# bootphon/abnet3

Hardware: AMD Instinct MI355X
Metric: frame-pairs/sec (Siamese train step: fwd both towers + coscos2 + bwd + Adadelta) (higher is better)
Workload: dtype f16x2; 1 GPU; C2: SiameseNetwork 40->500x2->100 sigmoid, coscos2(avg=False), Adadelta(0.1), 4096 frame pairs per GPU per step, 40-d N(0,1) frames; pairs_per_gpu=4096, global_pairs=4096, parallelism=dp1, graph_replay=False, dp_gradient_buckets=1

## Files before the change

### abnet3_amd/csrc/common.h

```cpp
#pragma once
#include <hip/hip_runtime.h>
#include <stdint.h>
#include <stdio.h>

#include "../../include/abnet3_hip.h"

namespace abn {

void set_error(const char* fmt, ...);

#define ABN_REQUIRE(cond, ...)                      \
    do {                                            \
        if (!(cond)) {                              \
            ::abn::set_error(__VA_ARGS__);          \
            return ABN_E_ARG;                       \
        }                                           \
    } while (0)

#define ABN_CHECK_LAUNCH(what)                                               \
    do {                                                                     \
        hipError_t e_ = hipGetLastError();                                   \
        if (e_ != hipSuccess) {                                              \
            ::abn::set_error("%s: %s", what, hipGetErrorString(e_));         \
            return ABN_E_LAUNCH;                                             \
// ... 3 lines not shown
struct Switches {
    bool planes;
    bool fused;
    int64_t fused_min_rows;
    bool bn_planes;
    bool bn_persist;
    bool wgrad_xcd;
    bool bf16x3_planes;
    bool bwd_pair;
    int gemm_tile;
    bool dtw_f40, dtw_pc;
    int wgrad_tile128;
    int dtw_wgs_per_cu;
    int wgrad_wgs_heavy, wgrad_wgs_light;
    int64_t wgrad_rows_per_slab;
    bool wide;
    int64_t wide_max_rows;
    int wide_max_groups;
    bool wgrad_step;
    bool dtw_dealt;
    int oneshot_wgs;
    int knn_split;
    int sd_tiles;
};
const Switches& switches();
void reload_switches();

__device__ __forceinline__ bool abn_ticket_publish(double* slot, double value, unsigned* counter, unsigned n_tickets)
{
    __hip_atomic_store(slot, value, __ATOMIC_RELAXED, __HIP_MEMORY_SCOPE_AGENT);
#ifdef ABN_STRICT_FENCES
    const unsigned ticket = __hip_atomic_fetch_add(counter, 1u, __ATOMIC_ACQ_REL, __HIP_MEMORY_SCOPE_AGENT);
#else
    __atomic_signal_fence(__ATOMIC_SEQ_CST);
    __builtin_amdgcn_s_waitcnt(0);
    __atomic_signal_fence(__ATOMIC_SEQ_CST);
    const unsigned ticket = __hip_atomic_fetch_add(counter, 1u, __ATOMIC_RELAXED, __HIP_MEMORY_SCOPE_AGENT);
#endif
    return ticket == n_tickets - 1;
}
__device__ __forceinline__ double abn_ticket_partial(const double* slot)
{
    return __hip_atomic_load(slot, __ATOMIC_RELAXED, __HIP_MEMORY_SCOPE_AGENT);
}

static inline int64_t align_up(int64_t v, int64_t a) { return (v + a - 1) / a * a; }
// ... 18 lines not shown
```

### abnet3_amd/csrc/tower.hip

```cpp
#include <stdarg.h>
#include <stdlib.h>
#include <string.h>

#include <math.h>
#include <atomic>

#include "common.h"
#include "gemm_f32.h"
#include "opt_rule.h"
#include "tower_fused.h"
#include "tower_planes.h"
#include "tower_bn_persist.h"
#include "tower_wide.h"
#include "tower_wgrad_step.h"

namespace abn {

static thread_local char g_err[512] = "";
void set_error(const char* fmt, ...)
{
    va_list ap;
    va_start(ap, fmt);
    vsnprintf(g_err, sizeof(g_err), fmt, ap);
    va_end(ap);
}

static Switches read_switches()
{
    auto off = [](const char* name) { const char* v = getenv(name); return v && atoi(v) == 0; };
    Switches s;
    s.planes = !off("ABN_PLANES");
    s.fused = !off("ABN_FUSED");
    s.fused_min_rows = getenv("ABN_FUSED_MIN_ROWS") ? atoll(getenv("ABN_FUSED_MIN_ROWS")) : -1;
// ... 3 lines not shown
    s.bf16x3_planes = !off("ABN_BF16X3_PLANES");
    s.bwd_pair = !off("ABN_BWD_PAIR");
    s.gemm_tile = getenv("ABN_GEMM_TILE") ? atoi(getenv("ABN_GEMM_TILE")) : -1;
    s.wgrad_rows_per_slab = getenv("ABN_WGRAD_ROWS_PER_SLAB") ? atoll(getenv("ABN_WGRAD_ROWS_PER_SLAB")) : -1;
    s.wide = !off("ABN_WIDE");
    s.wide_max_rows = getenv("ABN_WIDE_MAX_ROWS") ? atoll(getenv("ABN_WIDE_MAX_ROWS")) : -1;
    s.wide_max_groups = getenv("ABN_WIDE_MAXG") ? atoi(getenv("ABN_WIDE_MAXG")) : WD_MAXG;
    if (s.wide_max_groups < 1 || s.wide_max_groups > WD_MAXG) s.wide_max_groups = WD_MAXG;
    s.dtw_f40 = !off("ABN_DTW_F40");
    s.dtw_pc = !off("ABN_DTW_PC");
    s.wgrad_wgs_heavy = getenv("ABN_WGRAD_WGS_HEAVY") ? atoi(getenv("ABN_WGRAD_WGS_HEAVY")) : 128;
    s.wgrad_wgs_light = getenv("ABN_WGRAD_WGS_LIGHT") ? atoi(getenv("ABN_WGRAD_WGS_LIGHT")) : 128;
    s.wgrad_tile128 = getenv("ABN_WGRAD_TILE128") ? atoi(getenv("ABN_WGRAD_TILE128")) : -1;
    s.dtw_wgs_per_cu = getenv("ABN_DTW_WGS") ? atoi(getenv("ABN_DTW_WGS")) : 6;
    if (s.dtw_wgs_per_cu < 1 || s.dtw_wgs_per_cu > 9) s.dtw_wgs_per_cu = 6;
    s.wgrad_step = !off("ABN_WGRAD_STEP");
    s.dtw_dealt = !off("ABN_DTW_SCHED");
    s.oneshot_wgs = getenv("ABN_ONESHOT_WGS") ? atoi(getenv("ABN_ONESHOT_WGS")) : 32;
    if (s.oneshot_wgs < 1 || s.oneshot_wgs > 256) s.oneshot_wgs = 32;
    s.knn_split = getenv("ABN_KNN_SPLIT") ? atoi(getenv("ABN_KNN_SPLIT")) : 0;
    if (s.knn_split < 0) s.knn_split = 0;
    s.sd_tiles = getenv("ABN_SD_TILES") ? atoi(getenv("ABN_SD_TILES")) : 0;
    if (s.sd_tiles < 0 || s.sd_tiles > 4096) s.sd_tiles = 0;
    return s;
}
static Switches g_switches = read_switches();
const Switches& switches() { return g_switches; }
void reload_switches() { g_switches = read_switches(); }

#ifdef ABN_STAMPS
static unsigned long long* stamp_buffer(const char* name)
{
    const char* v = getenv(name);
    return v ? (unsigned long long*)strtoull(v, nullptr, 0) : nullptr;
}
#endif

template <int BM, int BN, bool A_KC, bool B_KC, int EPI, bool VEC, int BF16>
static void launch_one(const GemmP& p, int splits, hipStream_t st)
{
    const int tiles = ((p.M + BM - 1) / BM) * ((p.N + BN - 1) / BN);
    constexpr size_t lds = BF16 == 3 ? gemm_lds_bytes3<BM, BN>() : gemm_lds_bytes<BM, BN, A_KC, B_KC>();
    auto k = gemm_f32_kernel<BM, BN, A_KC, B_KC, EPI, VEC, BF16>;
    static bool attr_set[16] = {};
    if (first_use_on_device(attr_set))
        (void)hipFuncSetAttribute(reinterpret_cast<const void*>(k), hipFuncAttributeMaxDynamicSharedMemorySize, (int)lds);
// ... 154 lines not shown
    GemmP p = {};
    p.A = dz; p.lda = N;
    p.B = a_in; p.ldb = K;
    p.C = slabs; p.ldc = K;
    p.C2 = slabs + N * K;
    p.slab_stride = slab_stride;
    p.M = (int)N; p.N = (int)K + 1; p.K = (int)rows;
    p.k_chunk = (int)align_up((rows + splits - 1) / splits, BK);
    p.ones_col = (int)K;
    p.a_vec = vec_ok(dz, N);
    p.b_vec = vec_ok(a_in, K);
    p.bf16 = prec;
    return p;
}

__global__ void act_bwd_kernel(const float* __restrict__ a, const float* __restrict__ da,
                               const float* __restrict__ mask, float* __restrict__ dz, int64_t n, int act)
{
    for (int64_t i = blockIdx.x * (int64_t)blockDim.x + threadIdx.x; i < n;
         i += (int64_t)gridDim.x * blockDim.x)
        dz[i] = da[i] * act_grad(a[i], act) * (mask ? mask[i] : 1.0f);
}

struct ReduceTable {
    int n_layers;
    int splits[ABN_MAX_LAYERS];
    int64_t slab_stride;
    int64_t off[ABN_MAX_LAYERS];
    int64_t nW[ABN_MAX_LAYERS];
    int64_t nb[ABN_MAX_LAYERS];
    float* dW[ABN_MAX_LAYERS];
    float* db[ABN_MAX_LAYERS];
    int64_t total;
    int64_t begin;
    int n_extra;
    int64_t extra_off[2 * ABN_MAX_LAYERS];
    int32_t extra_n[2 * ABN_MAX_LAYERS];
    const unsigned* fail_word;
    int n_own;
    float* own[2 * ABN_MAX_LAYERS];
    int32_t own_n[2 * ABN_MAX_LAYERS];
};

__device__ __forceinline__ f32x4 sum_slabs(const float* __restrict__ src, int S, int64_t stride)
{
    f32x4 p[4] = {{0.f, 0.f, 0.f, 0.f}, {0.f, 0.f, 0.f, 0.f}, {0.f, 0.f, 0.f, 0.f}, {0.f, 0.f, 0.f, 0.f}};
    int k = 0;
    for (; k + 15 < S; k += 16) {
        f32x4 v[16];
#pragma unroll
        for (int u = 0; u < 16; ++u) v[u] = *reinterpret_cast<const f32x4*>(src + (int64_t)(k + u) * stride);
#pragma unroll
        for (int u = 0; u < 16; ++u) p[u & 3] += v[u];
    }
    for (; k + 3 < S; k += 4) {
        f32x4 v[4];
#pragma unroll
        for (int u = 0; u < 4; ++u) v[u] = *reinterpret_cast<const f32x4*>(src + (int64_t)(k + u) * stride);
#pragma unroll
        for (int u = 0; u < 4; ++u) p[u] += v[u];
    }
    for (; k < S; ++k) p[0] += *reinterpret_cast<const f32x4*>(src + (int64_t)k * stride);
    return (p[0] + p[1]) + (p[2] + p[3]);
}

__global__ void slab_reduce_kernel(const float* __restrict__ slabs, ReduceTable t)
{
    const bool dropped = t.fail_word && *t.fail_word != 0u;
    if (dropped && blockIdx.x == 0)
        for (int k = 0; k < t.n_own; ++k)
            for (int i = threadIdx.x; i < t.own_n[k]; i += blockDim.x) t.own[k][i] = 0.0f;
    const int64_t n4 = (t.total + 3) / 4;
    for (int64_t q = t.begin / 4 + blockIdx.x * (int64_t)blockDim.x + threadIdx.x; q < n4;
         q += (int64_t)gridDim.x * blockDim.x) {
        const int64_t i = 4 * q;
        int l = 0;
        while (l + 1 < t.n_layers && i >= t.off[l + 1]) ++l;
        const int S = t.splits[l];
        const f32x4 s = dropped ? f32x4{0.0f, 0.0f, 0.0f, 0.0f} : sum_slabs(slabs + i, S, t.slab_stride);
#pragma unroll
        for (int e = 0; e < 4; ++e) {
            const int64_t j = i + e - t.off[l];
            if (j < t.nW[l]) t.dW[l][j] = s[e];
            else if (j - t.nW[l] < t.nb[l]) t.db[l][j - t.nW[l]] = s[e];
        }
    }
}

__global__ void slab_reduce_step_kernel(const float* __restrict__ slabs, ReduceTable t, OptP o, float* __restrict__ params,
                                        float* __restrict__ grads, float* __restrict__ s1, float* __restrict__ s2,
                                        const unsigned* __restrict__ fail_word, int32_t* __restrict__ step_ctr)
{
    if (step_ctr && blockIdx.x == 0 && threadIdx.x == 0) *step_ctr += 1;
    if (fail_word && *fail_word != 0u) return;
    const int64_t n4 = (t.total + 3) / 4;
    for (int64_t q = blockIdx.x * (int64_t)blockDim.x + threadIdx.x; q < n4;
         q += (int64_t)gridDim.x * blockDim.x) {
        const int64_t i = 4 * q;
        int l = 0;
        while (l + 1 < t.n_layers && i >= t.off[l + 1]) ++l;
        const int S = t.splits[l];
        const int64_t baseW = t.dW[l] - grads, baseb = t.db[l] - grads;
        const int64_t j0 = i - t.off[l];
        const bool inW = j0 + 3 < t.nW[l], inb = j0 >= t.nW[l] && (j0 - t.nW[l]) + 3 < t.nb[l];
        const int64_t idx0 = inW ? baseW + j0 : baseb + (j0 - t.nW[l]);
        if ((inW || inb) && (idx0 & 3) == 0) {
            f32x4 pv = *reinterpret_cast<const f32x4*>(params + idx0);
            f32x4 av = *reinterpret_cast<const f32x4*>(s1 + idx0);
            f32x4 bv = {0.f, 0.f, 0.f, 0.f};
            if (opt_uses_s2(o)) bv = *reinterpret_cast<const f32x4*>(s2 + idx0);
            const f32x4 s = sum_slabs(slabs + i, S, t.slab_stride);
#pragma unroll
            for (int e = 0; e < 4; ++e) {
                float a1 = av[e], a2 = bv[e];
                pv[e] = opt_update_reg(o, pv[e], s[e], a1, a2);
                av[e] = a1; bv[e] = a2;
            }
            *reinterpret_cast<f32x4*>(grads + idx0) = s;
            *reinterpret_cast<f32x4*>(params + idx0) = pv;
            *reinterpret_cast<f32x4*>(s1 + idx0) = av;
            if (opt_uses_s2(o)) *reinterpret_cast<f32x4*>(s2 + idx0) = bv;
            continue;
        }
        const f32x4 s = sum_slabs(slabs + i, S, t.slab_stride);
#pragma unroll
        for (int e = 0; e < 4; ++e) {
            const int64_t j = j0 + e;
            int64_t idx;
            if (j < t.nW[l]) idx = baseW + j;
            else if (j - t.nW[l] < t.nb[l]) idx = baseb + (j - t.nW[l]);
            else continue;
            grads[idx] = s[e];
            params[idx] = opt_update(o, params[idx], s[e], s1, s2, idx);
        }
    }
    for (int x = 0; x < t.n_extra; ++x)
        for (int64_t j = blockIdx.x * (int64_t)blockDim.x + threadIdx.x; j < t.extra_n[x]; j += (int64_t)gridDim.x * blockDim.x) {
            const int64_t idx = t.extra_off[x] + j;
            params[idx] = opt_update(o, params[idx], grads[idx], s1, s2, idx);
        }
}


constexpr int BN_MAX_CHUNKS = 128;
static inline int bn_chunks(int64_t rows_per_call)
{
    const int64_t c = (rows_per_call + 63) / 64;
    return (int)(c < 1 ? 1 : (c > BN_MAX_CHUNKS ? BN_MAX_CHUNKS : c));
}
static inline int64_t bn_chunk_rows(int64_t rows_per_call) { return (rows_per_call + bn_chunks(rows_per_call) - 1) / bn_chunks(rows_per_call); }

template <bool BWD>
__global__ __launch_bounds__(256) void bn_partial_kernel(const float* __restrict__ z ,
                                                         const float* __restrict__ a, const float* __restrict__ xhat,
                                                         int64_t rows_per_call, int C, int64_t chunk_rows, int act,
                                                         double* __restrict__ part)
{
// ... 755 lines not shown
    ReduceTable rt = {};
    const int nl = t->n_layers;
    rt.n_layers = nl;
    rt.slab_stride = B.slab_stride;
    for (int l = 0; l < nl; ++l) {
        rt.splits[l] = B.splits[l];
        rt.off[l] = B.off[l];
        rt.nW[l] = t->dims[l + 1] * t->dims[l];
        rt.nb[l] = t->dims[l + 1];
        rt.dW[l] = t->dW[l];
        rt.db[l] = t->db[l];
    }
    rt.total = B.off[nl - 1] + rt.nW[nl - 1] + rt.nb[nl - 1];
    if (t->batch_norm && t->sync_ws) {
        rt.fail_word = reinterpret_cast<const unsigned*>(t->sync_ws) + 16;
        for (int l = 0; l < nl; ++l) {
            if (t->dbn_w[l]) { rt.own[rt.n_own] = t->dbn_w[l]; rt.own_n[rt.n_own++] = (int32_t)rt.nb[l]; }
            if (t->dbn_b[l]) { rt.own[rt.n_own] = t->dbn_b[l]; rt.own_n[rt.n_own++] = (int32_t)rt.nb[l]; }
        }
    }
    return rt;
}

static void reduce_one_layer(const float* slabs, int64_t slab_stride, int splits, int64_t in_dim, int64_t out_dim, float* dW, float* db,
                             hipStream_t st)
{
    ReduceTable rt = {};
    rt.n_layers = 1; rt.splits[0] = splits; rt.slab_stride = slab_stride;
    rt.off[0] = 0; rt.nW[0] = out_dim * in_dim; rt.nb[0] = out_dim; rt.dW[0] = dW; rt.db[0] = db;
    rt.total = out_dim * in_dim + out_dim;
    hipLaunchKernelGGL(slab_reduce_kernel, dim3(grid_for((rt.total + 3) / 4)), dim3(256), 0, st, slabs, rt);
}

static void bn_layer_backward(const abn_tower_desc* t, int l, int act, const float* da, float* dz, int64_t rows, int64_t n_calls,
                              const Layout& L, const BwdLayout& B, const float* ws, float* scratch, hipStream_t st)
{
    const int C = (int)t->dims[l + 1];
    const int64_t rpc = rows / n_calls;
    const float* a = ws + L.a[l];
    const int nch = bn_chunks(rpc);
    double* part = reinterpret_cast<double*>(scratch + B.bn_part);
    hipLaunchKernelGGL(bn_partial_kernel<true>, dim3((C + 63) / 64, nch, (int)n_calls), dim3(256), 0, st, da, a,
                       ws + L.xhat[l], rpc, C, bn_chunk_rows(rpc), act, part);
    hipLaunchKernelGGL(bn_bwd_finish_kernel, dim3((unsigned)((n_calls * C + 63) / 64)), dim3(64), 0, st, part,
                       nch, C, (int)n_calls, scratch + B.bn_s1, scratch + B.bn_s2);
    hipLaunchKernelGGL(bn_bwd_apply_kernel, dim3(grid_for(rows * C)), dim3(256), 0, st, a, da,
                       ws + L.xhat[l], rows, rpc, C, act, t->bn_w[l], ws + L.invstd[l], scratch + B.bn_s1, scratch + B.bn_s2,
                       (int)n_calls, t->drop_mask[l], dz, t->dbn_w[l], t->dbn_b[l]);
}

struct LossArgs {
    const void* y;
    int y_dtype, kind, avg;
    float margin;
// ... 45 lines not shown
    }
    *n_wg_out = n_wg;
    return w;
}

static int wgrad_range(const abn_tower_desc* t, int* l_first, int* l_end)
{
    *l_first = 0; *l_end = t->n_layers;
    if (t->wgrad_part == 0) return ABN_OK;
    ABN_REQUIRE(t->wgrad_part == 1 || t->wgrad_part == 2, "tower_backward: wgrad_part=%d", t->wgrad_part);
    ABN_REQUIRE(t->wgrad_split >= 0 && t->wgrad_split <= t->n_layers, "tower_backward: wgrad_split=%d", t->wgrad_split);
    ABN_REQUIRE(!t->defer_reduce, "tower_backward: wgrad_part cannot be combined with defer_reduce");
    if (t->wgrad_part == 1) *l_first = t->wgrad_split;
    else *l_end = t->wgrad_split;
    return ABN_OK;
}
static int reduce_slabs(const abn_tower_desc* t, const BwdLayout& B, const float* scratch, int l_first, int l_end, hipStream_t st)
{
    if (t->defer_reduce) return ABN_OK;
    ReduceTable rt = make_reduce_table(t, B);
    rt.begin = B.off[l_first < t->n_layers ? l_first : t->n_layers - 1];
    if (l_first >= t->n_layers) rt.begin = rt.total;
    if (l_end < t->n_layers) rt.total = B.off[l_end];
    if (rt.total > rt.begin)
        hipLaunchKernelGGL(slab_reduce_kernel, dim3(grid_for((rt.total - rt.begin + 3) / 4)), dim3(256), 0, st, scratch + B.slabs, rt);
    ABN_CHECK_LAUNCH("slab_reduce");
    return ABN_OK;
}

static int bn_planes_backward(const abn_tower_desc* t, const float* d_out, const LossArgs* loss, int64_t rows, int64_t n_calls, const Layout& L,
                              const BwdLayout& B0, const float* ws, float* scratch, float* dx, hipStream_t st)
{
    const int nl = t->n_layers;
    const int np = planes_of(t);
    const int64_t rpc = rows / n_calls;
    ABN_REQUIRE(aligned16(d_out) && aligned16(scratch) && (!dx || aligned16(dx)), "tower_backward: d_out / scratch / dx must be 16-byte aligned");
    ABN_REQUIRE(!t->d_out_is_dz || loss, "tower_backward: d_out_is_dz cannot be combined with batch_norm");
    ABN_REQUIRE(!loss || n_calls == 2, "tower_backward_loss: two forward_once calls");
    BwdLayout B = B0;
    for (int l = 0; l < nl; ++l) B.splits[l] = B0.psplits[l];
    const PackLayout PL = make_pack_layout(t);
    const char* const image = t->wpack ? reinterpret_cast<const char*>(t->wpack) : reinterpret_cast<const char*>(ws + L.wpack);
    static bool attr_set[16] = {};
    if (first_use_on_device(attr_set)) {
        PL_LDS_ATTR(bn_bwd_layer_kernel, pl_lds_bytes);
        PL_LDS_ATTR(wgrad_planes_kernel, wgrad_lds_of);
    }
    const int wgs_per_call = (int)bn_wgs_per_call(rows, n_calls);
// ... 256 lines not shown
                    q.y = t->source->labels;
                    q.g_steps = t->source->steps; q.g_ctr = t->source->step_ctr;
                }
            }
        }
        const dim3 grid((unsigned)(nrb * q.G));
        PL_LAUNCH(np, wide_dgrad_layer_kernel, grid, dim3(PL_NT), wd_lds_bytes(np), st, q);
        if (l < top || q.dz_out) cur ^= (q.dz_out ? 1 : 0);
        if (l == 0) break;
    }
    if (wgrad_step_small_ok(t, rows, n_calls)) {
        ABN_REQUIRE(t->fwd_ws == ws && t->fwd_calls == n_calls, "tower_backward: abn_tower_desc.fwd_ws / fwd_calls are not this call's");
        ABN_CHECK_LAUNCH("tower_backward (layer per launch)");
        return ABN_OK;
    }
    int n_wg = 0;
    WgradP w = make_wgrad(t, rows, L, B, ws, scratch, &n_wg, l_first, l_end);
    w.tp_steps = 2 * nrb;
    if (n_wg > 0) launch_wgrad(np, w, n_wg, st);
    ABN_CHECK_LAUNCH("tower_backward (layer per launch)");
    return reduce_slabs(t, B, scratch, l_first, l_end, st);
}

static int make_planes_fwd(const abn_tower_desc* t, const float* x1, const float* x2, int64_t rows, int64_t n_calls, int train,
                           const Layout& L, float* ws, hipStream_t st, PlanesFwdP* out)
{
    const int np = planes_of(t);
    PackTable pk = {};
    PlanesFwdP f = {};
    f.n_layers = t->n_layers;
    f.rows = (int)rows;
    f.rows_call = (int)(rows / n_calls);
    f.x1 = x1; f.x2 = x2;
    f.x_copy = nullptr;
    const PackLayout PL = make_pack_layout(t);
    char* const image = t->wpack ? reinterpret_cast<char*>(t->wpack) : reinterpret_cast<char*>(ws + L.wpack);
    const bool repack = !(t->wpack && t->wpack_valid);
    ABN_REQUIRE(aligned16(image), "tower_forward: wpack must be 16-byte aligned");
    pk.base = image;
    f.wbase = image; f.wbytes = PL.bytes;
    for (int l = 0; l <= t->n_layers; ++l) f.dims[l] = (int)t->dims[l];
    for (int l = 0; l < t->n_layers; ++l) {
        f.act[l] = (l == t->n_layers - 1) ? t->last_act : t->act;
        f.b[l] = t->b[l];
        f.mask[l] = train ? t->drop_mask[l] : nullptr;
        f.out[l] = l == t->n_layers - 1 ? ws + L.a[l] : nullptr;
        f.wp[l] = image + PL.wp[l];
        PackJob& J = pk.job[pk.n_jobs++];
        J.W = t->W[l]; J.N = (int)t->dims[l + 1]; J.K = (int)t->dims[l]; J.transposed = 0;
        J.nblk = pl_blocks(J.N); J.nsteps = pl_steps(J.K);
        J.tile0 = pk.n_tiles; J.dst = PL.wp[l];
        J.blk0 = pk.n_blocks;
        pk.n_tiles += J.nblk * J.nsteps;
        pk.n_blocks += J.nblk;
        {
            PackJob& T = pk.job[pk.n_jobs++];
            T.W = t->W[l]; T.N = J.N; T.K = J.K; T.transposed = 1;
            T.nblk = pl_blocks(T.K); T.nsteps = pl_steps(T.N);
            T.tile0 = pk.n_tiles; T.dst = PL.wpt[l];
            T.blk0 = pk.n_blocks;
            pk.n_tiles += T.nblk * T.nsteps;
            pk.n_blocks += T.nblk;
        }
        f.tp[l] = (t->forward_only || t->batch_norm) ? nullptr : reinterpret_cast<char*>(ws + L.tp[l]);
        f.amax[l] = f.tp[l] && L.amax[l] >= 0 ? ws + L.amax[l] : nullptr;
        if (t->batch_norm) { f.bn_rm[l] = t->bn_rm[l]; f.bn_rv[l] = t->bn_rv[l]; f.bn_w[l] = t->bn_w[l]; f.bn_b[l] = t->bn_b[l]; }
    }
    f.tp_steps = pl_row_steps(rows);
    f.drop_seed = train ? reinterpret_cast<const unsigned long long*>(t->drop_seed) : nullptr;
    f.drop_p = t->drop_p;
    f.bn_eps = BN_EPS;
#ifdef ABN_STAMPS
    f.stamps = stamp_buffer("ABN_STAMP_BUF");
#endif
    if (repack) {
        const dim3 pgrid((unsigned)((pk.n_tiles + 3) / 4));
        if (np == 3) hipLaunchKernelGGL(pack_planes_kernel<3>, pgrid, dim3(256), 0, st, pk);
        else if (np == 2) hipLaunchKernelGGL(pack_planes_scaled_kernel, dim3((unsigned)pk.n_blocks), dim3(PL_NT), 0, st, pk);
        else hipLaunchKernelGGL(pack_planes_kernel<1>, pgrid, dim3(256), 0, st, pk);
    }
    *out = f;
    return ABN_OK;
}

static int wide_forward(const abn_tower_desc* t, const float* x1, const float* x2, int64_t rows, int64_t n_calls, int train,
                        const Layout& L, float* ws, hipStream_t st)
{
    PlanesFwdP f;
    { const int rc = make_planes_fwd(t, x1, x2, rows, n_calls, train, L, ws, st, &f); if (rc != ABN_OK) return rc; }
    const int np = planes_of(t);
    static bool wd_attr_set[16] = {};
    if (first_use_on_device(wd_attr_set)) PL_LDS_ATTR(wide_fwd_layer_kernel, wd_lds_bytes);
    const int nl = t->n_layers;
    const int64_t wpc = bn_wgs_per_call(rows, n_calls), nrb = n_calls * wpc;
    const int G = wide_groups_for(t, nrb * PL_ROWS);
    const bool keep = !t->forward_only;
    for (int l = 0; l < nl; ++l) {
        WideFwdP q = {};
        q.l = l; q.last = l == nl - 1;
        q.K = (int)t->dims[l]; q.N = (int)t->dims[l + 1];
        q.act = f.act[l];
// ... 567 lines not shown
            if (hipFuncSetAttribute(reinterpret_cast<const void*>(wgrad_step_small_kernel), hipFuncAttributeMaxDynamicSharedMemorySize, (int)WGS_LDS_BYTES) != hipSuccess) {
                set_error("tower_reduce_step: cannot reserve %zu bytes of LDS", WGS_LDS_BYTES);
                return ABN_E_LAUNCH;
            }
            wgs_attr[dev] = true;
        }
        hipLaunchKernelGGL(wgrad_step_small_kernel, dim3((unsigned)n_wg), dim3(WGS_NT), WGS_LDS_BYTES, (hipStream_t)stream, w);
        ABN_CHECK_LAUNCH("tower_reduce_step (weight gradients + step)");
        return ABN_OK;
    }
    ReduceTable rt = make_reduce_table(t, B);
    for (int l = 0; l < t->n_layers; ++l) {
        ABN_REQUIRE(t->dW[l] && t->db[l] && t->dW[l] >= grads && t->dW[l] + rt.nW[l] <= grads + n && t->db[l] >= grads &&
                        t->db[l] + rt.nb[l] <= grads + n,
                    "tower_reduce_step: layer %d's gradients are not inside the flat buffer", l);
        if (t->batch_norm) {
            ABN_REQUIRE(t->dbn_w[l] && t->dbn_b[l] && t->dbn_w[l] >= grads && t->dbn_w[l] + rt.nb[l] <= grads + n &&
                            t->dbn_b[l] >= grads && t->dbn_b[l] + rt.nb[l] <= grads + n,
                        "tower_reduce_step: layer %d's BatchNorm gradients are not inside the flat buffer", l);
            rt.extra_off[rt.n_extra] = t->dbn_w[l] - grads; rt.extra_n[rt.n_extra++] = (int32_t)rt.nb[l];
            rt.extra_off[rt.n_extra] = t->dbn_b[l] - grads; rt.extra_n[rt.n_extra++] = (int32_t)rt.nb[l];
        }
    }
    hipLaunchKernelGGL(slab_reduce_step_kernel, dim3(grid_for((rt.total + 3) / 4)), dim3(256), 0, (hipStream_t)stream,
                       scratch + B.slabs, rt, make_optp(kind, lr, hp0, hp1, eps, step, grad_scale), params, grads, state1,
                       state2, t->batch_norm && t->sync_ws ? reinterpret_cast<const unsigned*>(t->sync_ws) + 16 : nullptr,
                       t->source ? t->source->step_ctr : nullptr);
    ABN_CHECK_LAUNCH("tower_reduce_step");
    return ABN_OK;
}


int abn_linear_forward(const float* x, const float* W, const float* b, int64_t rows, int64_t in_dim,
                       int64_t out_dim, int act, float* y, void* stream)
{
    ABN_REQUIRE(x && W && y, "linear_forward: null pointer");
    ABN_REQUIRE(rows >= 0 && rows < (1LL << 30) && in_dim >= 1 && out_dim >= 1 && in_dim < (1 << 24) && out_dim < (1 << 24),
                "linear_forward: bad shape");
    ABN_REQUIRE(act >= ABN_ACT_NONE && act <= ABN_ACT_TANH, "linear_forward: unsupported activation %d", act);
    const GemmP p = fwd_gemm(x, W, b, y, rows, in_dim, out_dim, act, nullptr, 0);
    return launch_gemm<true, true, EPI_FWD>(p, 1, (hipStream_t)stream);
}

int abn_linear_dgrad(const float* dz, const float* W, int64_t rows, int64_t in_dim, int64_t out_dim,
                     const float* a_prev, int act_prev, float* dx, void* stream)
{
    ABN_REQUIRE(dz && W && dx, "linear_dgrad: null pointer");
    ABN_REQUIRE(rows >= 0 && rows < (1LL << 30) && in_dim >= 1 && out_dim >= 1 && in_dim < (1 << 24) && out_dim < (1 << 24),
                "linear_dgrad: bad shape");
    ABN_REQUIRE(act_prev >= ABN_ACT_NONE && act_prev <= ABN_ACT_TANH, "linear_dgrad: unsupported activation %d", act_prev);
// ... 67 lines not shown
```

### abnet3_amd/csrc/tower_planes.h

```cpp
#pragma once
#include <type_traits>

#include "gemm_f32.h"

namespace abn {

typedef int v4i __attribute__((ext_vector_type(4)));

constexpr int PL_ROWS = 32;
constexpr int PL_WAVES = 8;
constexpr int PL_NT = 64 * PL_WAVES;
constexpr int PL_MAXW = 512;
constexpr int PL_MAXSTEPS = PL_MAXW / 16;
#ifdef PL_DEPTH_OVERRIDE
constexpr int PL_DEPTH = PL_DEPTH_OVERRIDE;
#else
constexpr int PL_DEPTH = 4;
#endif
constexpr int PL_PART_BYTES = 4 * 16 * 64 * 4;
constexpr int PL_SC_BYTES = PL_WAVES * 64 * 4 + PL_WAVES * 32 * 4;
constexpr int PL_AMAX = 32;

__host__ __device__ inline int pl_steps(int64_t contraction) { return ((int)((contraction + 15) / 16) + PL_DEPTH - 1) / PL_DEPTH * PL_DEPTH; }
__host__ __device__ inline int pl_blocks(int64_t features) { return (int)((features + 31) / 32); }
// ... 184 lines not shown
template <int NP>
__device__ __forceinline__ int tgather_row_offset(int r)
{
    const int sp = r >> 4, jh = (r >> 3) & 1, jl = r & 3, hp = (r >> 2) & 1;
    if constexpr (NP >= 2) return sp * 2048 + jh * 1024 + hp * 32 * 16 + jl * 4;
    else return sp * 1024 + hp * 32 * 16 + (4 * jh + jl) * 2;
}
template <int NP>
__device__ __forceinline__ float tgather(const char* tile_pair, int row_off, int c)
{
    if constexpr (NP >= 2) return *reinterpret_cast<const float*>(tile_pair + row_off + c * 16);
    else return (float)*reinterpret_cast<const __bf16*>(tile_pair + row_off + c * 16);
}

template <int N> __device__ __forceinline__ void wait_vmcnt() { asm volatile("s_waitcnt vmcnt(%0)" :: "n"(N) : "memory"); }

struct PackJob {
    const float* W;
    int N, K;
    int transposed;
    int nblk, nsteps;
    int tile0;
    int blk0;
    int64_t dst;
};
struct PackTable {
    int n_jobs, n_tiles, n_blocks;
    char* base;
    PackJob job[2 * ABN_MAX_LAYERS];
};

template <int NP>
__global__ __launch_bounds__(256) void pack_planes_kernel(PackTable t)
{
    const int tile = __builtin_amdgcn_readfirstlane(blockIdx.x * 4 + (threadIdx.x >> 6));
    if (tile >= t.n_tiles) return;
    const int lane = threadIdx.x & 63, r = lane & 31, h = lane >> 5;
    int jn = 0;
    while (jn + 1 < t.n_jobs && tile >= t.job[jn + 1].tile0) ++jn;
    const PackJob& J = t.job[jn];
    const int local = tile - J.tile0;
    const int nb = local / J.nsteps, s = local % J.nsteps;
    const int a = 32 * nb + r;
    const int rows_a = J.transposed ? J.K : J.N;
    const int len_c = J.transposed ? J.N : J.K;
    f32x4 v0 = {0.f, 0.f, 0.f, 0.f}, v1 = v0;
    if (a < rows_a) {
        const int c0 = 16 * s + 4 * h, c1 = c0 + 8;
        if (!J.transposed) {
            if (c0 < len_c) v0 = *reinterpret_cast<const f32x4*>(J.W + (int64_t)a * J.K + c0);
            if (c1 < len_c) v1 = *reinterpret_cast<const f32x4*>(J.W + (int64_t)a * J.K + c1);
        } else {
#pragma unroll
            for (int e = 0; e < 4; ++e) {
                if (c0 + e < len_c) v0[e] = J.W[(int64_t)(c0 + e) * J.K + a];
                if (c1 + e < len_c) v1[e] = J.W[(int64_t)(c1 + e) * J.K + a];
            }
        }
    }
    write_frag<NP>(t.base + J.dst + ((int64_t)local * NP) * 1024 + lane * 16, v0, v1);
}

__global__ __launch_bounds__(PL_NT) void pack_planes_scaled_kernel(PackTable t)
{
    __shared__ float wmax[PL_WAVES];
    const int lane = threadIdx.x & 63, r = lane & 31, h = lane >> 5;
    const int wave = __builtin_amdgcn_readfirstlane(threadIdx.x >> 6);
    const int b = blockIdx.x;
    int jn = 0;
    while (jn + 1 < t.n_jobs && b >= t.job[jn + 1].blk0) ++jn;
    const PackJob& J = t.job[jn];
    const int nb = b - J.blk0;
    const int rows_a = J.transposed ? J.K : J.N;
    const int len_c = J.transposed ? J.N : J.K;
    const int a = 32 * nb + r;
    const int ac = a < rows_a ? a : rows_a - 1;
    constexpr int SPW = PL_MAXSTEPS / PL_WAVES;
    f32x4 v[SPW][2];
    float m = 0.0f;
#pragma unroll
    for (int i = 0; i < SPW; ++i) {
        const int s = wave + PL_WAVES * i;
        const bool live = s < J.nsteps && a < rows_a;
#pragma unroll
        for (int u = 0; u < 2; ++u) {
            const int c = 16 * s + 4 * h + 8 * u;
            const int cc = c < len_c ? c : len_c - 4;
            f32x4 x;
            if (!J.transposed) {
                x = *reinterpret_cast<const f32x4*>(J.W + (int64_t)ac * J.K + cc);
            } else {
#pragma unroll
                for (int e = 0; e < 4; ++e) x[e] = J.W[(int64_t)(cc + e) * J.K + ac];
            }
            const bool ok = live && c < len_c;
#pragma unroll
            for (int e = 0; e < 4; ++e) v[i][u][e] = ok ? x[e] : 0.0f;
        }
        m = fmaxf(m, absmax8(v[i][0], v[i][1]));
    }
    m = wave_max(m);
    if (lane == 0) wmax[wave] = m;
    __syncthreads();
#pragma unroll
    for (int w = 0; w < PL_WAVES; ++w) m = fmaxf(m, wmax[w]);
    float sc, inv;
    scale_of(m, sc, inv);
    char* const image = t.base + J.dst;
#pragma unroll
    for (int i = 0; i < SPW; ++i) {
        const int s = wave + PL_WAVES * i;
        if (s < J.nsteps) write_frag<2>(image + ((int64_t)(nb * J.nsteps + s) * 2) * 1024 + lane * 16, v[i][0], v[i][1], sc);
    }
    if (threadIdx.x == 0) reinterpret_cast<float*>(image + (int64_t)J.nblk * J.nsteps * 2048)[nb] = inv;
}
__device__ __forceinline__ float packed_inv(const char* __restrict__ image, int nblk, int nsteps, int blk)
{
    return reinterpret_cast<const float*>(image + (int64_t)nblk * nsteps * 2048)[blk < nblk ? blk : nblk - 1];
}

#ifdef PL_HANDOVER_ON
constexpr bool PL_HANDOVER = true;
#else
constexpr bool PL_HANDOVER = false;
#endif
#ifndef PL_THROTTLE_LAG
#define PL_THROTTLE_LAG 0
#endif
#ifndef PL_THROTTLE_NAP
#define PL_THROTTLE_NAP 2
#endif
template <int NP>
struct WeightRing {
    __amdgpu_buffer_rsrc_t rs;
    v4i wq[PL_DEPTH][2][NP];
    bool filled;
};
// ... 1910 lines not shown
```

Measured before the change: 26.03 million frame-pairs/s.

## Rework slab reduction into per-wave chunks and split scaled weight packing across workgroups

The slab reduce and reduce+optimizer-step kernels now assign fixed 256-float chunks to waves. Segments are sorted by split count, and templated batch loads are specialized by slab count, so the per-element layer search goes away and loads can be issued together. The scaled weight-pack kernel is split into multiple workgroups per block. Its transposed path now reads coalesced rows and transposes through LDS, where it previously used strided scalar loads. Each part recomputes the full block absmax, which duplicates read work. Legacy paths and timing stamps remain available behind env switches.

```diff
diff --git a/abnet3_amd/csrc/common.h b/abnet3_amd/csrc/common.h
--- a/abnet3_amd/csrc/common.h
+++ b/abnet3_amd/csrc/common.h
@@ -49,6 +49,10 @@
     int oneshot_wgs;
     int knn_split;
     int sd_tiles;
+    bool pack_legacy;
+    int pack_split;
+    bool reduce_legacy;
+    int reduce_wgs;
 };
 const Switches& switches();
 void reload_switches();
diff --git a/abnet3_amd/csrc/tower.hip b/abnet3_amd/csrc/tower.hip
--- a/abnet3_amd/csrc/tower.hip
+++ b/abnet3_amd/csrc/tower.hip
@@ -9,6 +9,7 @@
 #include "gemm_f32.h"
 #include "opt_rule.h"
 #include "tower_fused.h"
+#include <climits>
 #include "tower_planes.h"
 #include "tower_bn_persist.h"
 #include "tower_wide.h"
@@ -58,6 +59,12 @@
     if (s.knn_split < 0) s.knn_split = 0;
     s.sd_tiles = getenv("ABN_SD_TILES") ? atoi(getenv("ABN_SD_TILES")) : 0;
     if (s.sd_tiles < 0 || s.sd_tiles > 4096) s.sd_tiles = 0;
+    s.pack_legacy = getenv("ABN_PACK_LEGACY") && atoi(getenv("ABN_PACK_LEGACY")) == 1;
+    s.pack_split = getenv("ABN_PACK_SPLIT") ? atoi(getenv("ABN_PACK_SPLIT")) : 4;
+    if (s.pack_split != 1 && s.pack_split != 2 && s.pack_split != 4) s.pack_split = 4;
+    s.reduce_legacy = getenv("ABN_REDUCE_LEGACY") && atoi(getenv("ABN_REDUCE_LEGACY")) == 1;
+    s.reduce_wgs = getenv("ABN_REDUCE_WGS") ? atoi(getenv("ABN_REDUCE_WGS")) : 4;
+    if (s.reduce_wgs < 1 || s.reduce_wgs > 16) s.reduce_wgs = 4;
     return s;
 }
 static Switches g_switches = read_switches();
@@ -258,6 +265,15 @@
         dz[i] = da[i] * act_grad(a[i], act) * (mask ? mask[i] : 1.0f);
 }
 
+struct ReduceSeg {
+    int64_t off;
+    int64_t nW, nb;
+    float* dW;
+    float* db;
+    int S;
+    int chunk0;
+    int64_t pad[2];
+};
 struct ReduceTable {
     int n_layers;
     int splits[ABN_MAX_LAYERS];
@@ -276,7 +292,20 @@
     int n_own;
     float* own[2 * ABN_MAX_LAYERS];
     int32_t own_n[2 * ABN_MAX_LAYERS];
+    int n_chunks;
+    int seg_first[ABN_MAX_LAYERS];
+    ReduceSeg seg[ABN_MAX_LAYERS];
+#ifdef ABN_STAMPS
+    unsigned long long* stamps;
+#endif
 };
+constexpr int RC_FLOATS = 256;
+#ifdef ABN_STAMPS
+#define RSTAMP(on, slot, drain) do { if ((on) && t.stamps && threadIdx.x == 0) { if (drain) asm volatile("s_waitcnt vmcnt(0)" ::: "memory"); \
+    t.stamps[(size_t)blockIdx.x * 8 + (slot)] = __builtin_amdgcn_s_memtime(); } } while (0)
+#else
+#define RSTAMP(on, slot, drain) do {} while (0)
+#endif
 
 __device__ __forceinline__ f32x4 sum_slabs(const float* __restrict__ src, int S, int64_t stride)
 {
@@ -300,33 +329,80 @@
     return (p[0] + p[1]) + (p[2] + p[3]);
 }
 
-__global__ void slab_reduce_kernel(const float* __restrict__ slabs, ReduceTable t)
+template <int SB>
+__device__ __forceinline__ f32x4 sum_batch(const float* __restrict__ src, unsigned lane_off, int S, int64_t stride)
+{
+    if constexpr (SB == 0) {
+        return sum_slabs(src + lane_off, S, stride);
+    } else {
+        f32x4 v[SB];
+#pragma unroll
+        for (int u = 0; u < SB; ++u) {
+            const float* const slab = src + (int64_t)(u < S ? u : (S > 0 ? S - 1 : 0)) * stride;
+            v[u] = *reinterpret_cast<const f32x4*>(&slab[lane_off]);
+        }
+        f32x4 p[4] = {{0.f, 0.f, 0.f, 0.f}, {0.f, 0.f, 0.f, 0.f}, {0.f, 0.f, 0.f, 0.f}, {0.f, 0.f, 0.f, 0.f}};
+        if (S == SB) {
+#pragma unroll
+            for (int u = 0; u < SB; ++u) p[u & 3] += v[u];
+        } else {
+            const int S4 = S & ~3;
+#pragma unroll
+            for (int u = 0; u < SB; ++u) {
+                if (u < S4) p[u & 3] += v[u];
+                else if (u < S) p[0] += v[u];
+            }
+        }
+        return (p[0] + p[1]) + (p[2] + p[3]);
+    }
+}
+
+__device__ __forceinline__ int segment_of(const ReduceTable& t, int c)
+{
+    int g = 0;
+#pragma unroll
+    for (int k = 1; k < ABN_MAX_LAYERS; ++k) g += c >= t.seg_first[k] ? 1 : 0;
+    return g;
+}
+
+template <int SB>
+__device__ __forceinline__ void reduce_chunk(const float* __restrict__ slabs, const ReduceSeg& sg, int64_t stride, bool dropped, int64_t c_off, unsigned lane_off)
+{
+    const int64_t nW = sg.nW, nb = sg.nb;
+    const int64_t j0 = c_off + lane_off;
+    if (j0 >= nW + nb) return;
+    const f32x4 s = dropped ? f32x4{0.0f, 0.0f, 0.0f, 0.0f} : sum_batch<SB>(slabs + sg.off + c_off, lane_off, sg.S, stride);
+#pragma unroll
+    for (int e = 0; e < 4; ++e) {
+        const int64_t j = j0 + e;
+        if (j < nW) sg.dW[j] = s[e];
+        else if (j - nW < nb) sg.db[j - nW] = s[e];
+    }
+}
+__global__ __launch_bounds__(256) void slab_reduce_kernel(const float* __restrict__ slabs, ReduceTable t)
 {
     const bool dropped = t.fail_word && *t.fail_word != 0u;
     if (dropped && blockIdx.x == 0)
         for (int k = 0; k < t.n_own; ++k)
             for (int i = threadIdx.x; i < t.own_n[k]; i += blockDim.x) t.own[k][i] = 0.0f;
-    const int64_t n4 = (t.total + 3) / 4;
-    for (int64_t q = t.begin / 4 + blockIdx.x * (int64_t)blockDim.x + threadIdx.x; q < n4;
-         q += (int64_t)gridDim.x * blockDim.x) {
-        const int64_t i = 4 * q;
-        int l = 0;
-        while (l + 1 < t.n_layers && i >= t.off[l + 1]) ++l;
-        const int S = t.splits[l];
-        const f32x4 s = dropped ? f32x4{0.0f, 0.0f, 0.0f, 0.0f} : sum_slabs(slabs + i, S, t.slab_stride);
-#pragma unroll
-        for (int e = 0; e < 4; ++e) {
-            const int64_t j = i + e - t.off[l];
-            if (j < t.nW[l]) t.dW[l][j] = s[e];
-            else if (j - t.nW[l] < t.nb[l]) t.db[l][j - t.nW[l]] = s[e];
-        }
-    }
-}
-
-__global__ void slab_reduce_step_kernel(const float* __restrict__ slabs, ReduceTable t, OptP o, float* __restrict__ params,
+    const int wave = __builtin_amdgcn_readfirstlane(threadIdx.x >> 6), lane = threadIdx.x & 63;
+    for (int c = blockIdx.x * 4 + wave; c < t.n_chunks; c += gridDim.x * 4) {
+        const ReduceSeg sg = t.seg[segment_of(t, c)];
+        const int64_t c_off = (int64_t)(c - sg.chunk0) * RC_FLOATS;
+        const int S = sg.S;
+        if (S > 32) reduce_chunk<0>(slabs, sg, t.slab_stride, dropped, c_off, 4u * lane);
+        else if (S > 16) reduce_chunk<32>(slabs, sg, t.slab_stride, dropped, c_off, 4u * lane);
+        else if (S > 8) reduce_chunk<16>(slabs, sg, t.slab_stride, dropped, c_off, 4u * lane);
+        else if (S > 4) reduce_chunk<8>(slabs, sg, t.slab_stride, dropped, c_off, 4u * lane);
+        else reduce_chunk<4>(slabs, sg, t.slab_stride, dropped, c_off, 4u * lane);
+    }
+}
+
+__global__ void slab_reduce_step_legacy_kernel(const float* __restrict__ slabs, ReduceTable t, OptP o, float* __restrict__ params,
                                         float* __restrict__ grads, float* __restrict__ s1, float* __restrict__ s2,
                                         const unsigned* __restrict__ fail_word, int32_t* __restrict__ step_ctr)
 {
+    RSTAMP(true, 0, false);
     if (step_ctr && blockIdx.x == 0 && threadIdx.x == 0) *step_ctr += 1;
     if (fail_word && *fail_word != 0u) return;
     const int64_t n4 = (t.total + 3) / 4;
@@ -345,7 +421,9 @@
             f32x4 av = *reinterpret_cast<const f32x4*>(s1 + idx0);
             f32x4 bv = {0.f, 0.f, 0.f, 0.f};
             if (opt_uses_s2(o)) bv = *reinterpret_cast<const f32x4*>(s2 + idx0);
+            RSTAMP(true, 1, true);
             const f32x4 s = sum_slabs(slabs + i, S, t.slab_stride);
+            RSTAMP(true, 2, true);
 #pragma unroll
             for (int e = 0; e < 4; ++e) {
                 float a1 = av[e], a2 = bv[e];
@@ -356,6 +434,7 @@
             *reinterpret_cast<f32x4*>(params + idx0) = pv;
             *reinterpret_cast<f32x4*>(s1 + idx0) = av;
             if (opt_uses_s2(o)) *reinterpret_cast<f32x4*>(s2 + idx0) = bv;
+            RSTAMP(true, 3, true);
             continue;
         }
         const f32x4 s = sum_slabs(slabs + i, S, t.slab_stride);
@@ -369,6 +448,81 @@
             grads[idx] = s[e];
             params[idx] = opt_update(o, params[idx], s[e], s1, s2, idx);
         }
+    }
+    for (int x = 0; x < t.n_extra; ++x)
+        for (int64_t j = blockIdx.x * (int64_t)blockDim.x + threadIdx.x; j < t.extra_n[x]; j += (int64_t)gridDim.x * blockDim.x) {
+            const int64_t idx = t.extra_off[x] + j;
+            params[idx] = opt_update(o, params[idx], grads[idx], s1, s2, idx);
+        }
+}
+
+template <int SB>
+__device__ __forceinline__ void reduce_step_chunk(const float* __restrict__ slabs, const ReduceTable& t, const ReduceSeg& sg, const OptP& o,
+                                                  float* __restrict__ params, float* __restrict__ grads, float* __restrict__ s1,
+                                                  float* __restrict__ s2, int64_t c_off, unsigned lane_off, bool first)
+{
+    const int64_t nW = sg.nW, nb = sg.nb;
+    const int S = sg.S;
+    const int64_t j0 = c_off + lane_off;
+    if (j0 >= nW + nb) return;
+    const float* const src = slabs + sg.off + c_off;
+    const int64_t baseW = sg.dW - grads, baseb = sg.db - grads;
+    const bool inW = j0 + 3 < nW, inb = j0 >= nW && (j0 - nW) + 3 < nb;
+    const int64_t idx0 = inW ? baseW + j0 : baseb + (j0 - nW);
+    if ((inW || inb) && (idx0 & 3) == 0) {
+        f32x4 pv = *reinterpret_cast<const f32x4*>(params + idx0);
+        f32x4 av = *reinterpret_cast<const f32x4*>(s1 + idx0);
+        f32x4 bv = {0.f, 0.f, 0.f, 0.f};
+        if (opt_uses_s2(o)) bv = *reinterpret_cast<const f32x4*>(s2 + idx0);
+        RSTAMP(first, 1, true);
+        const f32x4 s = sum_batch<SB>(src, lane_off, S, t.slab_stride);
+        RSTAMP(first, 2, true);
+#pragma unroll
+        for (int e = 0; e < 4; ++e) {
+            float a1 = av[e], a2 = bv[e];
+            pv[e] = opt_update_reg(o, pv[e], s[e], a1, a2);
+            av[e] = a1; bv[e] = a2;
+        }
+        *reinterpret_cast<f32x4*>(grads + idx0) = s;
+        *reinterpret_cast<f32x4*>(params + idx0) = pv;
+        *reinterpret_cast<f32x4*>(s1 + idx0) = av;
+        if (opt_uses_s2(o)) *reinterpret_cast<f32x4*>(s2 + idx0) = bv;
+        RSTAMP(first, 3, true);
+        return;
+    }
+    const f32x4 s = sum_batch<SB>(src, lane_off, S, t.slab_stride);
+#pragma unroll
+    for (int e = 0; e < 4; ++e) {
+        const int64_t j = j0 + e;
+        int64_t idx;
+        if (j < nW) idx = baseW + j;
+        else if (j - nW < nb) idx = baseb + (j - nW);
+        else continue;
+        grads[idx] = s[e];
+        params[idx] = opt_update(o, params[idx], s[e], s1, s2, idx);
+    }
+}
+__global__ __launch_bounds__(256) void slab_reduce_step_kernel(const float* __restrict__ slabs, ReduceTable t, OptP o, float* __restrict__ params,
+                                                               float* __restrict__ grads, float* __restrict__ s1, float* __restrict__ s2,
+                                                               const unsigned* __restrict__ fail_word, int32_t* __restrict__ step_ctr)
+{
+    RSTAMP(true, 0, false);
+    const int wave = __builtin_amdgcn_readfirstlane(threadIdx.x >> 6), lane = threadIdx.x & 63;
+    const int c0 = blockIdx.x * 4 + wave;
+    ReduceSeg sg = t.seg[segment_of(t, c0 < t.n_chunks ? c0 : 0)];
+    if (step_ctr && blockIdx.x == 0 && threadIdx.x == 0) *step_ctr += 1;
+    if (fail_word && *fail_word != 0u) return;
+    for (int c = c0; c < t.n_chunks;) {
+        const int64_t c_off = (int64_t)(c - sg.chunk0) * RC_FLOATS;
+        const bool first = c == c0 && wave == 0;
+        const int S = sg.S;
+        if (S > 32) reduce_step_chunk<0>(slabs, t, sg, o, params, grads, s1, s2, c_off, 4u * lane, first);
+        else if (S > 16) reduce_step_chunk<32>(slabs, t, sg, o, params, grads, s1, s2, c_off, 4u * lane, first);
+        else if (S > 8) reduce_step_chunk<16>(slabs, t, sg, o, params, grads, s1, s2, c_off, 4u * lane, first);
+        else if (S > 4) reduce_step_chunk<8>(slabs, t, sg, o, params, grads, s1, s2, c_off, 4u * lane, first);
+        else reduce_step_chunk<4>(slabs, t, sg, o, params, grads, s1, s2, c_off, 4u * lane, first);
+        c += gridDim.x * 4;
+        if (c < t.n_chunks) sg = t.seg[segment_of(t, c)];
     }
     for (int x = 0; x < t.n_extra; ++x)
         for (int64_t j = blockIdx.x * (int64_t)blockDim.x + threadIdx.x; j < t.extra_n[x]; j += (int64_t)gridDim.x * blockDim.x) {
@@ -1170,6 +1324,30 @@
     return rt;
 }
 
+static int plan_chunks(ReduceTable& rt)
+{
+    int order[ABN_MAX_LAYERS], n_seg = 0;
+    for (int l = 0; l < rt.n_layers; ++l)
+        if (rt.off[l] >= rt.begin && rt.off[l] < rt.total) order[n_seg++] = l;
+    for (int a = 1; a < n_seg; ++a)
+        for (int b = a; b > 0 && rt.splits[order[b]] > rt.splits[order[b - 1]]; --b) {
+            const int x = order[b]; order[b] = order[b - 1]; order[b - 1] = x;
+        }
+    int64_t n = 0;
+    for (int g = 0; g < ABN_MAX_LAYERS; ++g) {
+        rt.seg_first[g] = g < n_seg ? (int)n : INT_MAX;
+        if (g >= n_seg) continue;
+        const int l = order[g];
+        ReduceSeg& sg = rt.seg[g];
+        sg.off = rt.off[l]; sg.nW = rt.nW[l]; sg.nb = rt.nb[l]; sg.dW = rt.dW[l]; sg.db = rt.db[l];
+        sg.S = rt.splits[l]; sg.chunk0 = (int)n;
+        n += (rt.nW[l] + rt.nb[l] + RC_FLOATS - 1) / RC_FLOATS;
+    }
+    rt.n_chunks = (int)n;
+    const int64_t wgs = (n + 3) / 4, cap = 256 * (int64_t)switches().reduce_wgs;
+    return (int)(wgs < 1 ? 1 : (wgs > cap ? cap : wgs));
+}
+
 static void reduce_one_layer(const float* slabs, int64_t slab_stride, int splits, int64_t in_dim, int64_t out_dim, float* dW, float* db,
                              hipStream_t st)
 {
@@ -1177,7 +1355,8 @@
     rt.n_layers = 1; rt.splits[0] = splits; rt.slab_stride = slab_stride;
     rt.off[0] = 0; rt.nW[0] = out_dim * in_dim; rt.nb[0] = out_dim; rt.dW[0] = dW; rt.db[0] = db;
     rt.total = out_dim * in_dim + out_dim;
-    hipLaunchKernelGGL(slab_reduce_kernel, dim3(grid_for((rt.total + 3) / 4)), dim3(256), 0, st, slabs, rt);
+    const int grid = plan_chunks(rt);
+    hipLaunchKernelGGL(slab_reduce_kernel, dim3(grid), dim3(256), 0, st, slabs, rt);
 }
 
 static void bn_layer_backward(const abn_tower_desc* t, int l, int act, const float* da, float* dz, int64_t rows, int64_t n_calls,
@@ -1269,8 +1448,10 @@
     rt.begin = B.off[l_first < t->n_layers ? l_first : t->n_layers - 1];
     if (l_first >= t->n_layers) rt.begin = rt.total;
     if (l_end < t->n_layers) rt.total = B.off[l_end];
-    if (rt.total > rt.begin)
-        hipLaunchKernelGGL(slab_reduce_kernel, dim3(grid_for((rt.total - rt.begin + 3) / 4)), dim3(256), 0, st, scratch + B.slabs, rt);
+    if (rt.total > rt.begin) {
+        const int grid = plan_chunks(rt);
+        hipLaunchKernelGGL(slab_reduce_kernel, dim3(grid), dim3(256), 0, st, scratch + B.slabs, rt);
+    }
     ABN_CHECK_LAUNCH("slab_reduce");
     return ABN_OK;
 }
@@ -1573,6 +1754,13 @@
     return reduce_slabs(t, B, scratch, l_first, l_end, st);
 }
 
+static int pack_parts(int nsteps, int split)
+{
+    const int per_part = PL_WAVES * (PL_MAXSTEPS / PL_WAVES) / split;
+    const int parts = (nsteps + per_part - 1) / per_part;
+    return parts < 1 ? 1 : (parts > split ? split : parts);
+}
+
 static int make_planes_fwd(const abn_tower_desc* t, const float* x1, const float* x2, int64_t rows, int64_t n_calls, int train,
                            const Layout& L, float* ws, hipStream_t st, PlanesFwdP* out)
 {
@@ -1589,6 +1777,10 @@
     const bool repack = !(t->wpack && t->wpack_valid);
     ABN_REQUIRE(aligned16(image), "tower_forward: wpack must be 16-byte aligned");
     pk.base = image;
+    pk.split = switches().pack_split;
+#ifdef ABN_STAMPS
+    pk.stamps = stamp_buffer("ABN_PSTAMP_BUF");
+#endif
     f.wbase = image; f.wbytes = PL.bytes;
     for (int l = 0; l <= t->n_layers; ++l) f.dims[l] = (int)t->dims[l];
     for (int l = 0; l < t->n_layers; ++l) {
@@ -1602,16 +1794,20 @@
         J.nblk = pl_blocks(J.N); J.nsteps = pl_steps(J.K);
         J.tile0 = pk.n_tiles; J.dst = PL.wp[l];
         J.blk0 = pk.n_blocks;
+        J.wg0 = pk.n_wgs; J.parts = pack_parts(J.nsteps, pk.split);
         pk.n_tiles += J.nblk * J.nsteps;
         pk.n_blocks += J.nblk;
+        pk.n_wgs += J.nblk * J.parts;
         {
             PackJob& T = pk.job[pk.n_jobs++];
             T.W = t->W[l]; T.N = J.N; T.K = J.K; T.transposed = 1;
             T.nblk = pl_blocks(T.K); T.nsteps = pl_steps(T.N);
             T.tile0 = pk.n_tiles; T.dst = PL.wpt[l];
             T.blk0 = pk.n_blocks;
+            T.wg0 = pk.n_wgs; T.parts = pack_parts(T.nsteps, pk.split);
             pk.n_tiles += T.nblk * T.nsteps;
             pk.n_blocks += T.nblk;
+            pk.n_wgs += T.nblk * T.parts;
         }
         f.tp[l] = (t->forward_only || t->batch_norm) ? nullptr : reinterpret_cast<char*>(ws + L.tp[l]);
         f.amax[l] = f.tp[l] && L.amax[l] >= 0 ? ws + L.amax[l] : nullptr;
@@ -1624,10 +1820,12 @@
 #ifdef ABN_STAMPS
     f.stamps = stamp_buffer("ABN_STAMP_BUF");
 #endif
+    for (int k = 0; k < 2 * ABN_MAX_LAYERS; ++k) pk.wg_first[k] = k < pk.n_jobs ? pk.job[k].wg0 : INT_MAX;
     if (repack) {
         const dim3 pgrid((unsigned)((pk.n_tiles + 3) / 4));
         if (np == 3) hipLaunchKernelGGL(pack_planes_kernel<3>, pgrid, dim3(256), 0, st, pk);
-        else if (np == 2) hipLaunchKernelGGL(pack_planes_scaled_kernel, dim3((unsigned)pk.n_blocks), dim3(PL_NT), 0, st, pk);
+        else if (np == 2 && switches().pack_legacy) hipLaunchKernelGGL(pack_planes_scaled_legacy_kernel, dim3((unsigned)pk.n_blocks), dim3(PL_NT), 0, st, pk);
+        else if (np == 2) hipLaunchKernelGGL(pack_planes_scaled_kernel, dim3((unsigned)pk.n_wgs), dim3(PL_NT), 0, st, pk);
         else hipLaunchKernelGGL(pack_planes_kernel<1>, pgrid, dim3(256), 0, st, pk);
     }
     *out = f;
@@ -2241,10 +2439,20 @@
             rt.extra_off[rt.n_extra] = t->dbn_b[l] - grads; rt.extra_n[rt.n_extra++] = (int32_t)rt.nb[l];
         }
     }
-    hipLaunchKernelGGL(slab_reduce_step_kernel, dim3(grid_for((rt.total + 3) / 4)), dim3(256), 0, (hipStream_t)stream,
-                       scratch + B.slabs, rt, make_optp(kind, lr, hp0, hp1, eps, step, grad_scale), params, grads, state1,
-                       state2, t->batch_norm && t->sync_ws ? reinterpret_cast<const unsigned*>(t->sync_ws) + 16 : nullptr,
-                       t->source ? t->source->step_ctr : nullptr);
+    const unsigned* const fail_word = t->batch_norm && t->sync_ws ? reinterpret_cast<const unsigned*>(t->sync_ws) + 16 : nullptr;
+    int32_t* const step_ctr = t->source ? t->source->step_ctr : nullptr;
+    const int grid = plan_chunks(rt);
+#ifdef ABN_STAMPS
+    rt.stamps = stamp_buffer("ABN_RSTAMP_BUF");
+#endif
+    if (switches().reduce_legacy)
+        hipLaunchKernelGGL(slab_reduce_step_legacy_kernel, dim3(grid_for((rt.total + 3) / 4)), dim3(256), 0, (hipStream_t)stream,
+                           scratch + B.slabs, rt, make_optp(kind, lr, hp0, hp1, eps, step, grad_scale), params, grads, state1,
+                           state2, fail_word, step_ctr);
+    else
+        hipLaunchKernelGGL(slab_reduce_step_kernel, dim3(grid), dim3(256), 0, (hipStream_t)stream,
+                           scratch + B.slabs, rt, make_optp(kind, lr, hp0, hp1, eps, step, grad_scale), params, grads, state1,
+                           state2, fail_word, step_ctr);
     ABN_CHECK_LAUNCH("tower_reduce_step");
     return ABN_OK;
 }
diff --git a/abnet3_amd/csrc/tower_planes.h b/abnet3_amd/csrc/tower_planes.h
--- a/abnet3_amd/csrc/tower_planes.h
+++ b/abnet3_amd/csrc/tower_planes.h
@@ -230,13 +230,26 @@
     int nblk, nsteps;
     int tile0;
     int blk0;
+    int wg0, parts;
     int64_t dst;
 };
 struct PackTable {
     int n_jobs, n_tiles, n_blocks;
+    int n_wgs, split;
+    int wg_first[2 * ABN_MAX_LAYERS];
     char* base;
+#ifdef ABN_STAMPS
+    unsigned long long* stamps;
+#endif
     PackJob job[2 * ABN_MAX_LAYERS];
 };
+
+#ifdef ABN_STAMPS
+#define KSTAMP(slot, drain) do { if (t.stamps && threadIdx.x == 0) { if (drain) asm volatile("s_waitcnt vmcnt(0)" ::: "memory"); \
+    t.stamps[(size_t)blockIdx.x * 8 + (slot)] = __builtin_amdgcn_s_memtime(); } } while (0)
+#else
+#define KSTAMP(slot, drain) do {} while (0)
+#endif
 
 template <int NP>
 __global__ __launch_bounds__(256) void pack_planes_kernel(PackTable t)
@@ -269,9 +282,10 @@
     write_frag<NP>(t.base + J.dst + ((int64_t)local * NP) * 1024 + lane * 16, v0, v1);
 }
 
-__global__ __launch_bounds__(PL_NT) void pack_planes_scaled_kernel(PackTable t)
+__global__ __launch_bounds__(PL_NT) void pack_planes_scaled_legacy_kernel(PackTable t)
 {
     __shared__ float wmax[PL_WAVES];
+    KSTAMP(0, false);
     const int lane = threadIdx.x & 63, r = lane & 31, h = lane >> 5;
     const int wave = __builtin_amdgcn_readfirstlane(threadIdx.x >> 6);
     const int b = blockIdx.x;
@@ -307,9 +321,11 @@
         }
         m = fmaxf(m, absmax8(v[i][0], v[i][1]));
     }
+    KSTAMP(1, true);
     m = wave_max(m);
     if (lane == 0) wmax[wave] = m;
     __syncthreads();
+    KSTAMP(2, false);
 #pragma unroll
     for (int w = 0; w < PL_WAVES; ++w) m = fmaxf(m, wmax[w]);
     float sc, inv;
@@ -321,6 +337,96 @@
         if (s < J.nsteps) write_frag<2>(image + ((int64_t)(nb * J.nsteps + s) * 2) * 1024 + lane * 16, v[i][0], v[i][1], sc);
     }
     if (threadIdx.x == 0) reinterpret_cast<float*>(image + (int64_t)J.nblk * J.nsteps * 2048)[nb] = inv;
+    KSTAMP(3, true);
+}
+constexpr int PK_LD = 36;
+__global__ __launch_bounds__(PL_NT) void pack_planes_scaled_kernel(PackTable t)
+{
+    __shared__ float wmax[PL_WAVES];
+    __shared__ __attribute__((aligned(16))) float ttile[PL_WAVES][16 * PK_LD];
+    KSTAMP(0, false);
+    const int lane = threadIdx.x & 63, r = lane & 31, h = lane >> 5;
+    const int wave = __builtin_amdgcn_readfirstlane(threadIdx.x >> 6);
+    const int g = blockIdx.x;
+    int jn = 0;
+#pragma unroll
+    for (int k = 1; k < 2 * ABN_MAX_LAYERS; ++k) jn += g >= t.wg_first[k] ? 1 : 0;
+    const PackJob J = t.job[jn];
+    const int nb = (g - J.wg0) % J.nblk, part = (g - J.wg0) / J.nblk;
+    const int rows_a = J.transposed ? J.K : J.N;
+    const int len_c = J.transposed ? J.N : J.K;
+    constexpr int SPW = PL_MAXSTEPS / PL_WAVES;
+    f32x4 v[SPW][2];
+    float m = 0.0f;
+    if (!J.transposed) {
+        const int a = 32 * nb + r;
+        const int ac = a < rows_a ? a : rows_a - 1;
+#pragma unroll
+        for (int i = 0; i < SPW; ++i) {
+            const int s = wave + PL_WAVES * i;
+            const bool live = s < J.nsteps && a < rows_a;
+#pragma unroll
+            for (int u = 0; u < 2; ++u) {
+                const int c = 16 * s + 4 * h + 8 * u;
+                const int cc = c < len_c ? c : len_c - 4;
+                const f32x4 x = *reinterpret_cast<const f32x4*>(J.W + (int64_t)ac * J.K + cc);
+                const bool ok = live && c < len_c;
+#pragma unroll
+                for (int e = 0; e < 4; ++e) v[i][u][e] = ok ? x[e] : 0.0f;
+            }
+        }
+    } else {
+        const int k = 32 * nb + 4 * (lane & 7);
+        const int kc = k < rows_a ? k : rows_a - 4;
+#pragma unroll
+        for (int i = 0; i < SPW; ++i) {
+            const int s = wave + PL_WAVES * i;
+#pragma unroll
+            for (int u = 0; u < 2; ++u) {
+                const int n = 16 * s + (lane >> 3) + 8 * u;
+                const int nc = n < len_c ? n : len_c - 1;
+                const f32x4 x = *reinterpret_cast<const f32x4*>(J.W + (int64_t)nc * J.K + kc);
+                const bool ok = s < J.nsteps && n < len_c && k < rows_a;
+#pragma unroll
+                for (int e = 0; e < 4; ++e) v[i][u][e] = ok ? x[e] : 0.0f;
+            }
+        }
+    }
+#pragma unroll
+    for (int i = 0; i < SPW; ++i) m = fmaxf(m, absmax8(v[i][0], v[i][1]));
+    KSTAMP(1, true);
+    m = wave_max(m);
+    if (lane == 0) wmax[wave] = m;
+    __syncthreads();
+    KSTAMP(2, false);
+#pragma unroll
+    for (int w = 0; w < PL_WAVES; ++w) m = fmaxf(m, wmax[w]);
+    float sc, inv;
+    scale_of(m, sc, inv);
+    char* const image = t.base + J.dst;
+    float* const T = ttile[wave];
+#pragma unroll
+    for (int i = 0; i < SPW; ++i) {
+        const int s = wave + PL_WAVES * i;
+        if (i * t.split / SPW != part || s >= J.nsteps) continue;
+        f32x4 w0 = v[i][0], w1 = v[i][1];
+        if (J.transposed) {
+            *reinterpret_cast<f32x4*>(T + (lane >> 3) * PK_LD + 4 * (lane & 7)) = w0;
+            *reinterpret_cast<f32x4*>(T + ((lane >> 3) + 8) * PK_LD + 4 * (lane & 7)) = w1;
+            __builtin_amdgcn_fence(__ATOMIC_ACQ_REL, "workgroup");
+            __builtin_amdgcn_wave_barrier();
+#pragma unroll
+            for (int e = 0; e < 4; ++e) {
+                w0[e] = T[(4 * h + e) * PK_LD + r];
+                w1[e] = T[(4 * h + 8 + e) * PK_LD + r];
+            }
+            __builtin_amdgcn_fence(__ATOMIC_ACQ_REL, "workgroup");
+            __builtin_amdgcn_wave_barrier();
+        }
+        write_frag<2>(image + ((int64_t)(nb * J.nsteps + s) * 2) * 1024 + lane * 16, w0, w1, sc);
+    }
+    if (threadIdx.x == 0 && part == 0) reinterpret_cast<float*>(image + (int64_t)J.nblk * J.nsteps * 2048)[nb] = inv;
+    KSTAMP(3, true);
 }
 __device__ __forceinline__ float packed_inv(const char* __restrict__ image, int nblk, int nsteps, int blk)
 {
```

After: 25.86 million frame-pairs/s. No clear change (-0.6%).
